# IST-DASLab/gptq-gguf-toolkit

Measured on AMD Instinct MI355X. Metric: Mparams/s GPTQ-quantized, higher is better.
Workload: dtype f32; 1 GPU; llama3-8b-block-q4k: 7 Linears of one block (218.1 M params), 128x2048-token calibration fed per sequence through the package's BlockSchedule, block_size 128, rel_damp 0.01, nstep 20; calib_seqs_per_rank=128, parallelism=calib-dp1+matrix-fanout, owners=rank0

## Files before the change

### gptq-gguf-toolkit_amd/csrc/gq_gemm3p.hpp

```cpp
#pragma once
#include <algorithm>
#include <atomic>
#include <vector>

#include "gq_common.hpp"

namespace gq {
namespace p3 {

constexpr int BLK = 8192;
constexpr int TILE = 256;
constexpr int SLOT_BYTES = 4 * BLK;
constexpr int LDS_BYTES = 4 * SLOT_BYTES;
constexpr int CPT = 8;
typedef float f32x4 __attribute__((ext_vector_type(4)));
typedef unsigned u32x4 __attribute__((ext_vector_type(4)));

__host__ __device__ __forceinline__ unsigned swz(int r) { return (0x78u >> (2 * ((r >> 2) & 3))) & 3u; }

__device__ __forceinline__ void split3(const float (&x)[8], uint4& p1, uint4& p2, uint4& p3) {
    unsigned a[8], b[8], c[8];
#pragma unroll
    for (int e = 0; e < 8; ++e) {
        const unsigned xb = __builtin_bit_cast(unsigned, x[e]);
        const unsigned x1 = xb & 0xffff0000u;
        const float xr = x[e] - __builtin_bit_cast(float, x1);
        const unsigned x2 = __builtin_bit_cast(unsigned, xr) & 0xffff0000u;
        const float xs = xr - __builtin_bit_cast(float, x2);
        a[e] = x1; b[e] = x2; c[e] = __builtin_bit_cast(unsigned, xs);
    }
    p1 = make_uint4(__builtin_amdgcn_perm(a[1], a[0], 0x07060302u), __builtin_amdgcn_perm(a[3], a[2], 0x07060302u),
                    __builtin_amdgcn_perm(a[5], a[4], 0x07060302u), __builtin_amdgcn_perm(a[7], a[6], 0x07060302u));
    p2 = make_uint4(__builtin_amdgcn_perm(b[1], b[0], 0x07060302u), __builtin_amdgcn_perm(b[3], b[2], 0x07060302u),
                    __builtin_amdgcn_perm(b[5], b[4], 0x07060302u), __builtin_amdgcn_perm(b[7], b[6], 0x07060302u));
    p3 = make_uint4(__builtin_amdgcn_perm(c[1], c[0], 0x07060302u), __builtin_amdgcn_perm(c[3], c[2], 0x07060302u),
                    __builtin_amdgcn_perm(c[5], c[4], 0x07060302u), __builtin_amdgcn_perm(c[7], c[6], 0x07060302u));
}
__device__ __forceinline__ float scale_from_max(unsigned maxbits, float& inv) {
    const int ex = (int)((maxbits >> 23) & 0xff);
    int e = (ex == 0 || ex == 0xff) ? 0 : 14 - (ex - 127);
    e = e > 100 ? 100 : (e < -100 ? -100 : e);
    inv = __builtin_bit_cast(float, (unsigned)(127 - e) << 23);
    return __builtin_bit_cast(float, (unsigned)(127 + e) << 23);
}
__device__ __forceinline__ void split2h(const float (&x)[8], float mult, uint4& p1, uint4& p2) {
    unsigned a[4], b[4];
#pragma unroll
    for (int e = 0; e < 4; ++e) {
        unsigned lo[2], hi[2];
#pragma unroll
        for (int u = 0; u < 2; ++u) {
            float v = x[2 * e + u] * mult;
            asm volatile("" : "+v"(v));
            const _Float16 h1 = (_Float16)v;
            float r = v - (float)h1;
            asm volatile("" : "+v"(r));
            const _Float16 h2 = (_Float16)r;
            lo[u] = (unsigned)__builtin_bit_cast(uint16_t, h1);
            hi[u] = (unsigned)__builtin_bit_cast(uint16_t, h2);
        }
        a[e] = lo[0] | (lo[1] << 16);
        b[e] = hi[0] | (hi[1] << 16);
    }
    p1 = make_uint4(a[0], a[1], a[2], a[3]);
    p2 = make_uint4(b[0], b[1], b[2], b[3]);
}

template <int NP, bool TRANS>
__global__ __launch_bounds__(256) void split_kernel(const float* __restrict__ S, int64_t ld, int KC, int tri, int rev,
                                                    unsigned char* __restrict__ img, const unsigned* __restrict__ rmax,
                                                    float* __restrict__ inv_scale) {
    __shared__ float T[TRANS ? 32 : 1][TRANS ? 132 : 1];
    const int c = blockIdx.x, pn = blockIdx.y, tid = threadIdx.x;
    const int kblk = c >> 2;
    const bool zero = (tri == 1 && kblk > pn) || (tri == 2 && kblk < pn);
    if constexpr (TRANS) {
        if (!zero) {
#pragma unroll
            for (int u = 0; u < 4; ++u) {
                const int idx = tid + u * 256, kk = idx >> 5, r4 = (idx & 31) * 4;
                const float4 v = *reinterpret_cast<const float4*>(S + (int64_t)(32 * c + kk) * ld + 128 * pn + r4);
                T[kk][r4] = v.x; T[kk][r4 + 1] = v.y; T[kk][r4 + 2] = v.z; T[kk][r4 + 3] = v.w;
            }
        }
        __syncthreads();
    }
    unsigned char* out = img + ((size_t)pn * KC + (rev ? KC - 1 - c : c)) * (size_t)(NP * BLK);
#pragma unroll
    for (int u = 0; u < 2; ++u) {
        const int p = tid + u * 256, r = p >> 2, kc = (p & 3) ^ (int)swz(r);
        float x[8];
        if (zero) {
#pragma unroll
            for (int e = 0; e < 8; ++e) x[e] = 0.0f;
        } else if constexpr (TRANS) {
#pragma unroll
            for (int e = 0; e < 8; ++e) x[e] = T[8 * kc + e][r];
        } else {
            const float* src = S + (int64_t)(128 * pn + r) * ld + 32 * c + 8 * kc;
            const float4 v0 = *reinterpret_cast<const float4*>(src), v1 = *reinterpret_cast<const float4*>(src + 4);
            x[0] = v0.x; x[1] = v0.y; x[2] = v0.z; x[3] = v0.w; x[4] = v1.x; x[5] = v1.y; x[6] = v1.z; x[7] = v1.w;
        }
        if constexpr (NP == 3) {
            uint4 p1, p2, p3;
            split3(x, p1, p2, p3);
            *reinterpret_cast<uint4*>(out + p * 16) = p1;
            *reinterpret_cast<uint4*>(out + BLK + p * 16) = p2;
            *reinterpret_cast<uint4*>(out + 2 * BLK + p * 16) = p3;
        } else {
            float inv;
            const float mult = scale_from_max(rmax[128 * pn + r], inv);
            if (c == 0 && (p & 3) == 0) inv_scale[128 * pn + r] = inv;
            uint4 p1, p2;
            split2h(x, mult, p1, p2);
            *reinterpret_cast<uint4*>(out + p * 16) = p1;
            *reinterpret_cast<uint4*>(out + BLK + p * 16) = p2;
        }
    }
}

template <bool TRANS>
__global__ __launch_bounds__(256) void row_absmax_kernel(const float* __restrict__ S, int64_t ld, int tri,
                                                         unsigned* __restrict__ rmax) {
    const int kb = blockIdx.x, pn = blockIdx.y, tid = threadIdx.x;
    if ((tri == 1 && kb > pn) || (tri == 2 && kb < pn)) return;
    __shared__ unsigned part[128];
    if (tid < 128) part[tid] = 0u;
    __syncthreads();
    if constexpr (TRANS) {
        float m0 = 0.f, m1 = 0.f, m2 = 0.f, m3 = 0.f;
        const int r4 = (tid & 31) * 4;
#pragma unroll 4
        for (int kk = tid >> 5; kk < 128; kk += 8) {
            const float4 v = *reinterpret_cast<const float4*>(S + (int64_t)(128 * kb + kk) * ld + 128 * pn + r4);
            m0 = fmaxf(m0, fabsf(v.x)); m1 = fmaxf(m1, fabsf(v.y)); m2 = fmaxf(m2, fabsf(v.z)); m3 = fmaxf(m3, fabsf(v.w));
        }
        atomicMax(&part[r4], __builtin_bit_cast(unsigned, m0));
        atomicMax(&part[r4 + 1], __builtin_bit_cast(unsigned, m1));
        atomicMax(&part[r4 + 2], __builtin_bit_cast(unsigned, m2));
        atomicMax(&part[r4 + 3], __builtin_bit_cast(unsigned, m3));
    } else {
        const int r = tid >> 1, h = tid & 1;
        const float* src = S + (int64_t)(128 * pn + r) * ld + 128 * kb + 64 * h;
        float m = 0.f;
#pragma unroll 4
        for (int q = 0; q < 16; ++q) {
            const float4 v = *reinterpret_cast<const float4*>(src + 4 * q);
            m = fmaxf(m, fmaxf(fmaxf(fabsf(v.x), fabsf(v.y)), fmaxf(fabsf(v.z), fabsf(v.w))));
        }
        atomicMax(&part[r], __builtin_bit_cast(unsigned, m));
    }
    __syncthreads();
    if (tid < 128 && part[tid]) atomicMax(&rmax[128 * pn + tid], part[tid]);
}

struct Problem {
    const unsigned char* Aimg;
    const unsigned char* Bimg;
    uint32_t a_panel_bytes, b_panel_bytes;
    float* C;
    int64_t ldc;
    int mode;
    const float* row_scale;
    const float* col_scale;
    float* partial;
};
struct Group {
    Problem p[2];
    const uint32_t* table;
};
constexpr int T_UNITS = 260, NWG = 256;

template <int NP>
__global__ __launch_bounds__(512, 2) void gemm_kernel(const Group g) {
    extern __shared__ __attribute__((aligned(16))) unsigned char smem[];
    const int tid = threadIdx.x, lane = tid & 63;
    const int wid = __builtin_amdgcn_readfirstlane(tid >> 6);
    const int wm = wid >> 2, wn = wid & 3;
    const unsigned qb = g.table[blockIdx.x], qe = g.table[blockIdx.x + 1];
    const unsigned lds0 = (unsigned)(uintptr_t)smem;
    const unsigned ldsw = lds0 + (unsigned)wid * 1024u;
    const int lr = lane & 15, lk = lane >> 4;
    unsigned bA0, bA1, bB0, bB1;
    {
        const unsigned ch = ((unsigned)lk ^ swz(lr)) << 4;
        bA0 = lds0 + (unsigned)(wm * 128 + lr) * 64u + ch;
        bB0 = lds0 + 16384u + (unsigned)(wn * 64 + lr) * 64u + ch;
        bA1 = bA0 + 65536u;
        bB1 = bB0 + 65536u;
    }
    for (unsigned ui = qb; ui < qe; ++ui) {
        __syncthreads();
        const uint32_t* uw = g.table + T_UNITS + 4 * (size_t)ui;
        const uint32_t w0 = (uint32_t)__builtin_amdgcn_readfirstlane((int)uw[0]);
        const int cb = __builtin_amdgcn_readfirstlane((int)uw[1]), ce = __builtin_amdgcn_readfirstlane((int)uw[2]);
        const uint32_t w3 = (uint32_t)__builtin_amdgcn_readfirstlane((int)uw[3]);
        const Problem& P = g.p[w0 >> 28];
        const int tm = (int)((w0 >> 14) & 0x3fff), tn = (int)(w0 & 0x3fff);
        const char* a0 = reinterpret_cast<const char*>(P.Aimg) + (size_t)(2 * tm) * P.a_panel_bytes;
        const char* a1 = a0 + P.a_panel_bytes;
        const char* b0 = reinterpret_cast<const char*>(P.Bimg) + (size_t)(2 * tn) * P.b_panel_bytes;
        const char* b1 = b0 + P.b_panel_bytes;
        const char *a0p0 = a0, *a0p1 = a0 + BLK, *a1p0 = a1, *a1p1 = a1 + BLK;
        const char *b0p0 = b0, *b0p1 = b0 + BLK, *b1p0 = b1, *b1p1 = b1 + BLK;
        const char *a0p2 = a0 + 2 * BLK, *a1p2 = a1 + 2 * BLK, *b0p2 = b0 + 2 * BLK, *b1p2 = b1 + 2 * BLK;
        (void)a0p2; (void)a1p2; (void)b0p2; (void)b1p2;
        constexpr unsigned CH = NP * BLK;
        const unsigned vlast = (unsigned)(ce - 1) * CH + (unsigned)tid * 16u;
        unsigned V0 = (unsigned)cb * CH + (unsigned)tid * 16u, V1, V2, V3, V4;
#define P3_VNEXT()                                               \
    V1 = V0 + CH < vlast ? V0 + CH : vlast;                      \
    V2 = V0 + 2 * CH < vlast ? V0 + 2 * CH : vlast;              \
    V3 = V0 + 3 * CH < vlast ? V0 + 3 * CH : vlast;              \
    V4 = V0 + 4 * CH < vlast ? V0 + 4 * CH : vlast
        P3_VNEXT();
        (void)V3; (void)V4;
#define P3_DL(vo, sp, slot, part)                                                     \
    asm volatile("s_mov_b32 m0, %2\n\ts_nop 0\n\tglobal_load_lds_dwordx4 %0, %1"      \
                 :: "v"(vo), "s"(sp), "s"(ldsw + (unsigned)((slot) * SLOT_BYTES + (part) * BLK)) : "memory")
#define P3_DL4(vo, PA, PB, slot)                                                      \
    P3_DL(vo, a0p##PA, slot, 0); P3_DL(vo, a1p##PA, slot, 1); P3_DL(vo, b0p##PB, slot, 2); P3_DL(vo, b1p##PB, slot, 3)
        f32x4 c00, c01, c02, c03, c10, c11, c12, c13, c20, c21, c22, c23, c30, c31, c32, c33, c40, c41, c42, c43, c50,
            c51, c52, c53, c60, c61, c62, c63, c70, c71, c72, c73;
#define P3_Z(c) c = f32x4{0.f, 0.f, 0.f, 0.f}
        P3_Z(c00); P3_Z(c01); P3_Z(c02); P3_Z(c03); P3_Z(c10); P3_Z(c11); P3_Z(c12); P3_Z(c13);
        P3_Z(c20); P3_Z(c21); P3_Z(c22); P3_Z(c23); P3_Z(c30); P3_Z(c31); P3_Z(c32); P3_Z(c33);
        P3_Z(c40); P3_Z(c41); P3_Z(c42); P3_Z(c43); P3_Z(c50); P3_Z(c51); P3_Z(c52); P3_Z(c53);
        P3_Z(c60); P3_Z(c61); P3_Z(c62); P3_Z(c63); P3_Z(c70); P3_Z(c71); P3_Z(c72); P3_Z(c73);
#undef P3_Z
        u32x4 pa0, pa1, pa2, pa3, pa4, pa5, pa6, pa7, pb0, pb1, pb2, pb3;
        u32x4 qa0, qa1, qa2, qa3, qa4, qa5, qa6, qa7, qb0, qb1, qb2, qb3;
#define P3_DSR(dst, base, off) asm volatile("ds_read_b128 %0, %1 offset:%2" : "=v"(dst) : "v"(base), "n"(off) : "memory")
#define P3_LGKM1(N, x) asm volatile("s_waitcnt lgkmcnt(" #N ")" : "+v"(x)::"memory")
#define P3_LGKM2(N, x, y) asm volatile("s_waitcnt lgkmcnt(" #N ")" : "+v"(x), "+v"(y)::"memory")
#define P3_MF(c, a, b)                                                                                          \
    do {                                                                                                        \
        if constexpr (NP == 3) asm volatile("v_mfma_f32_16x16x32_bf16 %0, %1, %2, %0" : "+v"(c) : "v"(a), "v"(b)); \
        else asm volatile("v_mfma_f32_16x16x32_f16 %0, %1, %2, %0" : "+v"(c) : "v"(a), "v"(b));                 \
    } while (0)
#define P3_STEP(X, Y, AY, BY, OFF, MID, L0, L1, L2, L3)                                               \
    do {                                                                                              \
        P3_LGKM2(10, X##a0, X##b0);                                                                   \
        P3_MF(c00, X##a0, X##b0);                                                                     \
        MID;                                                                                          \
        P3_LGKM1(9, X##b1);                                                                           \
        P3_MF(c01, X##a0, X##b1);                                                                     \
        P3_DSR(Y##a0, AY, (OFF) + 0);                                                                 \
        P3_LGKM1(9, X##b2);                                                                           \
        P3_MF(c02, X##a0, X##b2);                                                                     \
        P3_LGKM1(8, X##b3);                                                                           \
        P3_MF(c03, X##a0, X##b3);                                                                     \
        P3_DSR(Y##b0, BY, (OFF) + 0);                                                                 \
        P3_LGKM1(8, X##a1);                                                                           \
        P3_MF(c10, X##a1, X##b0);                                                                     \
        P3_MF(c11, X##a1, X##b1);                                                                     \
        P3_DSR(Y##b1, BY, (OFF) + 1024);                                                              \
        P3_MF(c12, X##a1, X##b2);                                                                     \
        P3_MF(c13, X##a1, X##b3);                                                                     \
        P3_DSR(Y##b2, BY, (OFF) + 2048);                                                              \
        P3_LGKM1(9, X##a2);                                                                           \
        P3_MF(c20, X##a2, X##b0);                                                                     \
        P3_MF(c21, X##a2, X##b1);                                                                     \
        P3_DSR(Y##b3, BY, (OFF) + 3072);                                                              \
        P3_MF(c22, X##a2, X##b2);                                                                     \
        P3_MF(c23, X##a2, X##b3);                                                                     \
        P3_DSR(Y##a1, AY, (OFF) + 1024);                                                              \
        P3_LGKM1(10, X##a3);                                                                          \
        P3_MF(c30, X##a3, X##b0);                                                                     \
        P3_MF(c31, X##a3, X##b1);                                                                     \
        P3_DSR(Y##a2, AY, (OFF) + 2048);                                                              \
        L0;                                                                                           \
        P3_MF(c32, X##a3, X##b2);                                                                     \
        P3_MF(c33, X##a3, X##b3);                                                                     \
        P3_DSR(Y##a3, AY, (OFF) + 3072);                                                              \
        P3_LGKM1(11, X##a4);                                                                          \
        P3_MF(c40, X##a4, X##b0);                                                                     \
        P3_MF(c41, X##a4, X##b1);                                                                     \
        P3_DSR(Y##a4, AY, (OFF) + 4096);                                                              \
        L1;                                                                                           \
        P3_MF(c42, X##a4, X##b2);                                                                     \
        P3_MF(c43, X##a4, X##b3);                                                                     \
        P3_DSR(Y##a5, AY, (OFF) + 5120);                                                              \
        P3_LGKM1(12, X##a5);                                                                          \
        P3_MF(c50, X##a5, X##b0);                                                                     \
        P3_MF(c51, X##a5, X##b1);                                                                     \
        P3_DSR(Y##a6, AY, (OFF) + 6144);                                                              \
        L2;                                                                                           \
        P3_MF(c52, X##a5, X##b2);                                                                     \
        P3_MF(c53, X##a5, X##b3);                                                                     \
        P3_DSR(Y##a7, AY, (OFF) + 7168);                                                              \
        P3_LGKM1(13, X##a6);                                                                          \
        P3_MF(c60, X##a6, X##b0);                                                                     \
        P3_MF(c61, X##a6, X##b1);                                                                     \
        L3;                                                                                           \
        P3_MF(c62, X##a6, X##b2);                                                                     \
        P3_MF(c63, X##a6, X##b3);                                                                     \
        P3_LGKM1(12, X##a7);                                                                          \
        P3_MF(c70, X##a7, X##b0);                                                                     \
        P3_MF(c71, X##a7, X##b1);                                                                     \
        P3_MF(c72, X##a7, X##b2);                                                                     \
        P3_MF(c73, X##a7, X##b3);                                                                     \
    } while (0)
#define P3_IV0(VO, PA, PB)                                                                                        \
    P3_STEP(p, q, bA0, bB0, 32768, asm volatile("s_waitcnt vmcnt(4)\n\ts_barrier" ::: "memory"), P3_DL(VO, a0p##PA, 3, 0), \
            P3_DL(VO, a1p##PA, 3, 1), P3_DL(VO, b0p##PB, 3, 2), P3_DL(VO, b1p##PB, 3, 3))
#define P3_IV1(VO, PA, PB)                                                                                        \
// ... 166 lines not shown
    const int slot_base = 0;
    struct Tile { int prob, tm, tn, len; };
    std::vector<Tile> tiles;
    struct Blk { int neg_len, prob, bi, bj; };
    std::vector<Blk> blocks;
    for (int prob = 0; prob < (int)shapes.size(); ++prob) {
        const GemmShape& s = shapes[prob];
        const bool by_m = s.kr == 3;
        const int bm = by_m ? 4 : 8, bn = by_m ? 8 : 4;
        const int nbm = (s.MT + bm - 1) / bm, nbn = (s.NT + bn - 1) / bn;
        for (int bi = 0; bi < nbm; ++bi)
            for (int bj = 0; bj < nbn; ++bj) {
                int mx = 0;
                for (int tm = bi * bm; tm < std::min(s.MT, (bi + 1) * bm); ++tm)
                    for (int tn = bj * bn; tn < std::min(s.NT, (bj + 1) * bn); ++tn)
                        if (!s.lower || tm >= tn) mx = std::max(mx, tile_len(s, tm, tn));
                if (mx > 0) blocks.push_back({-mx, prob, bi, bj});
            }
    }
    std::stable_sort(blocks.begin(), blocks.end(), [](const Blk& a, const Blk& b) { return a.neg_len < b.neg_len; });
    for (auto& b : blocks) {
        const GemmShape& s = shapes[b.prob];
        const bool by_m = s.kr == 3;
        const int bm = by_m ? 4 : 8, bn = by_m ? 8 : 4;
        for (int tm = b.bi * bm; tm < std::min(s.MT, (b.bi + 1) * bm); ++tm)
            for (int tn = b.bj * bn; tn < std::min(s.NT, (b.bj + 1) * bn); ++tn)
                if (!s.lower || tm >= tn) {
                    const int len = tile_len(s, tm, tn);
                    if (len > 0) tiles.push_back({b.prob, tm, tn, len});
                }
    }
    struct Piece { int tile, cb, ce; };
    long total = 0;
    for (auto& t : tiles) total += t.len + OVH;
    std::vector<Piece> seg[8];
    {
        long acc = 0;
        int x = 0;
        for (int ti = 0; ti < (int)tiles.size(); ++ti) {
            int at = 0;
            const int len = tiles[ti].len;
            while (at < len) {
                const long end_x = (x == 7) ? (long)1 << 60 : (total * (x + 1)) / 8;
                long room = end_x - acc - OVH;
                int take = len - at;
                if (room < take) {
                    int r = (int)std::max<long>(room, 0) / gran * gran;
                    if (r < MINP) r = 0;
                    if (take - r < MINP) r = take;
                    take = r;
                }
                if (take > 0) {
                    seg[x].push_back({ti, at, at + take});
                    acc += take + OVH;
                    at += take;
                }
                if (at < len || acc >= end_x) {
                    if (x < 7) ++x;
                    else if (take == 0) { seg[x].push_back({ti, at, len}); acc += len - at + OVH; at = len; }
                }
            }
        }
    }
    std::vector<Piece> wg[NWG];
    double mk = 0;
    for (int x = 0; x < 8; ++x) {
        long tot = 0;
        for (auto& p : seg[x]) tot += p.ce - p.cb + OVH;
        std::vector<Piece> mine[32];
        long load[32];
        for (long T = (tot + 31) / 32;; T += gran) {
            for (int w = 0; w < 32; ++w) { load[w] = 0; mine[w].clear(); }
            size_t done = 0;
            while (done + 32 <= seg[x].size()) {
                bool ok = true;
                for (int w = 0; w < 32 && ok; ++w) {
                    const Piece& p = seg[x][done + w];
                    ok = load[w] + (p.ce - p.cb) + OVH <= T;
                }
                if (!ok) break;
                for (int w = 0; w < 32; ++w) {
                    const Piece& p = seg[x][done + w];
                    load[w] += p.ce - p.cb + OVH;
                    mine[w].push_back(p);
                }
                done += 32;
            }
            int w = 0;
            bool fits = true;
            for (size_t i = done; i < seg[x].size() && fits; ++i) {
                Piece p = seg[x][i];
                while (p.cb < p.ce) {
                    if (w > 31) { fits = false; break; }
                    const int len = p.ce - p.cb;
                    const long room = T - load[w] - OVH;
                    int take;
                    if (room >= len) take = len;
                    else {
                        take = (int)(std::max<long>(room, 0) / gran * gran);
                        if (len - take < MINP) take = (len - MINP) / gran * gran;
                        if (take < MINP) { ++w; continue; }
                    }
                    mine[w].push_back({p.tile, p.cb, p.cb + take});
                    load[w] += take + OVH;
                    p.cb += take;
                }
            }
            if (fits) break;
        }
        for (int w = 0; w < 32; ++w) {
            wg[w * 8 + x] = mine[w];
            mk = std::max(mk, (double)load[w]);
        }
    }
    std::vector<int> npieces(tiles.size(), 0), first_slot(tiles.size(), -1), seen(tiles.size(), 0);
    for (int b = 0; b < NWG; ++b)
        for (auto& p : wg[b]) ++npieces[p.tile];
    Plan pl;
    int slots = 0;
    for (size_t t = 0; t < tiles.size(); ++t)
        if (npieces[t] > 1) {
            first_slot[t] = slot_base + slots;
            slots += npieces[t];
            pl.rlist.push_back((uint32_t)tiles[t].prob << 28 | (uint32_t)tiles[t].tm << 14 | (uint32_t)tiles[t].tn);
            pl.rlist.push_back((uint32_t)first_slot[t] << 8 | (uint32_t)npieces[t]);
        }
    pl.nslots = slots;
    pl.table.assign(T_UNITS, 0u);
    unsigned at = 0;
    for (int b = 0; b < NWG; ++b) {
        pl.table[b] = at;
        for (auto& p : wg[b]) {
            const Tile& t = tiles[p.tile];
            pl.table.push_back((uint32_t)t.prob << 28 | (uint32_t)t.tm << 14 | (uint32_t)t.tn);
            pl.table.push_back((uint32_t)p.cb);
            pl.table.push_back((uint32_t)p.ce);
            pl.table.push_back(npieces[p.tile] > 1 ? (uint32_t)(first_slot[p.tile] + seen[p.tile]++ + 1) : 0u);
            ++at;
        }
    }
    pl.table[NWG] = at;
    pl.makespan = mk;
    pl.ideal = (double)total / NWG;
    if (slots > max_slots) pl.nslots = -1;
    return pl;
}

template <int NP>
inline int launch_split(bool trans, const float* S, int64_t ld, int64_t R, int64_t K, int tri, int rev, unsigned char* img,
                        unsigned* rmax, float* inv_scale, hipStream_t st) {
    const dim3 grid((unsigned)(K / 32), (unsigned)(R / 128)), block(256);
    ProfScope ps(PT_CHOL_SPLIT, st);
    if constexpr (NP == 2) {
        GQ_HIP(hipMemsetAsync(rmax, 0, (size_t)R * 4, st));
        const dim3 g2((unsigned)(K / 128), (unsigned)(R / 128));
        if (trans) hipLaunchKernelGGL(row_absmax_kernel<true>, g2, block, 0, st, S, ld, tri, rmax);
        else hipLaunchKernelGGL(row_absmax_kernel<false>, g2, block, 0, st, S, ld, tri, rmax);
        GQ_LAUNCH_CHECK();
    }
    if (trans) hipLaunchKernelGGL((split_kernel<NP, true>), grid, block, 0, st, S, ld, (int)(K / 32), tri, rev, img, rmax, inv_scale);
    else hipLaunchKernelGGL((split_kernel<NP, false>), grid, block, 0, st, S, ld, (int)(K / 32), tri, rev, img, rmax, inv_scale);
    GQ_LAUNCH_CHECK();
    return GQ_OK;
}

template <int NP>
inline int launch_gemm(const Group& g, int n_reduce, const uint32_t* rlist_dev, hipStream_t st) {
    static std::atomic<bool> attr_set{false};
    if (!attr_set) {
        GQ_HIP(hipFuncSetAttribute((const void*)gemm_kernel<NP>, hipFuncAttributeMaxDynamicSharedMemorySize, LDS_BYTES));
        attr_set = true;
    }
    ProfScope ps(PT_CHOL_IMG_GEMM, st);
    hipLaunchKernelGGL(gemm_kernel<NP>, dim3(256), dim3(512), LDS_BYTES, st, g);
    GQ_LAUNCH_CHECK();
    if (n_reduce > 0) {
        hipLaunchKernelGGL(reduce_kernel<NP>, dim3((unsigned)n_reduce, 16), dim3(256), 0, st, g, rlist_dev);
        GQ_LAUNCH_CHECK();
    }
    return GQ_OK;
}

}
}
```

### gptq-gguf-toolkit_amd/csrc/gq_gptq.hip

```cpp
#include <atomic>
#include <mutex>
#include "gq_common.hpp"
#include "gq_gemm32.hpp"
#include "gq_walk.hpp"
#include <stdlib.h>

namespace gq {

constexpr int SEG = 128;
constexpr int SB = 16;
constexpr int SEG_WAVES = 8;
constexpr int SEG_LDS_BYTES = (SEG * 64 + SEG * SEG + 2 * SB * 64) * 4 + SEG * 8;

__device__ __forceinline__ float div_rcp64(float n, double rd) { return (float)((double)n * rd); }

struct BandTable {
    int32_t n;
    int32_t end64[GQ_BANDS_MAX];
    uint32_t info[GQ_BANDS_MAX];
    int64_t sm_off[GQ_BANDS_MAX];
};
template <bool BANDS> struct BandArg {};
template <> struct BandArg<true> { BandTable t; };

// ... 476 lines not shown
    case WalkKind::Bands:
        hipLaunchKernelGGL((gptq_segment_kernel<false, false, true>), grid, block, SEG_LDS_BYTES, c.st, c.W, c.C, src, ld_src,
                           c.U, a, len, c.R, c.d, c.s, c.dmin, c.m, 0, 0, 0.0f, 0.0f, c.qweight, b.Err, ldE, err_col0, nullptr,
                           nullptr, nullptr, unext, npair, BandArg<true>{c.bands->tbl});
        break;
    case WalkKind::Uniform:
        hipLaunchKernelGGL((gptq_segment_kernel<false, true>), grid, block, SEG_LDS_BYTES, c.st, c.W, c.C, src, ld_src, c.U, a,
                           len, c.R, c.d, c.s, c.dmin, c.m, ti.group, 0, 0.0f, (float)ti.qmax, c.qweight, b.Err, ldE, err_col0,
                           nullptr, c.uni.scale, c.uni.zero, unext);
        break;
    case WalkKind::ActOrder:
        hipLaunchKernelGGL(gptq_segment_kernel<true>, grid, block, SEG_LDS_BYTES, c.st, c.W, c.C, src, ld_src, c.U, a, len, c.R,
                           c.d, c.s, c.dmin, c.m, ti.group, ti.is_signed, (float)ti.qmin, (float)ti.qmax, c.qweight, b.Err, ldE,
                           err_col0, c.perm, nullptr, nullptr, unext, npair);
        break;
    case WalkKind::KQuant:
        hipLaunchKernelGGL(gptq_segment_kernel<false>, grid, block, SEG_LDS_BYTES, c.st, c.W, c.C, src, ld_src, c.U, a, len, c.R,
                           c.d, c.s, c.dmin, c.m, ti.group, ti.is_signed, (float)ti.qmin, (float)ti.qmax, c.qweight, b.Err, ldE,
                           err_col0, nullptr, nullptr, nullptr, unext, npair);
        break;
    }
    GQ_LAUNCH_CHECK();
    return GQ_OK;
}

static int walk_block(const Walk& w, const Block& b, bool& walked_by_partner) {
    const WalkCall& c = w.c;
    const int64_t B = w.p.B;
    int rc;
    if (!b.single) {
        ProfScope ps(PT_BLOCK_FAR, c.st);
        hipLaunchKernelGGL(copy2d_kernel, dim3(2048), dim3(256), 0, c.st, w.Wblk, B, c.W + b.c1, c.C, c.R, b.c2 - b.c1);
        GQ_LAUNCH_CHECK();
    }
    int64_t a = walked_by_partner ? b.c2 : b.c1;
    walked_by_partner = false;
    while (a < b.c2) {
        int64_t e = a + SEG < b.c2 ? a + SEG : b.c2;
        const int64_t next_sg = (a / 256 + 1) * 256;
        if (e > next_sg) e = next_sg;
        const int len = (int)(e - a);
        if (w.search == ScaleSearch::Lazy && (a % 256) == 0 && (rc = lazy_search(w, a))) return rc;
        const float* unext =
            (w.p.pair_look && b.single && len == SEG && !(b.pos & 1) && b.c2 + B <= c.C) ? c.U + a * c.C + a + SEG : nullptr;
        const int npair = (unext && c.kind != WalkKind::Uniform && B == SEG) ? 2 : 1;
        walked_by_partner = npair == 2;
        if ((rc = launch_segment(w, b, a, len, unext, npair))) return rc;
        if (e < b.c2) {
            ProfScope ps(PT_BLOCK_FAR, c.st);
            hipLaunchKernelGGL(block_far_update_kernel, dim3(2048), dim3(256), 0, c.st, w.Wblk + (e - b.c1), B, b.c2 - e, c.R,
                               b.Err, w.p.ldE, a - b.c1, len, c.U, c.C, a, e);
            GQ_LAUNCH_CHECK();
        }
        a = e;
    }
    return GQ_OK;
}


static int block_trailing_update(const Walk& w, const Block& b, int64_t end) {
    const WalkCall& c = w.c;
    return launch_trailing_update(c.W + b.c2, c.C, b.Err + b.pos * w.p.B, w.p.ldE, c.U + b.c1 * c.C + b.c2, c.C, c.R,
                                  end - b.c2, b.c2 - b.c1, c.st);
}

static int pair_near_update(const Walk& w, const Block& b) {
    if (!(b.pos & 1)) return GQ_OK;
    const WalkCall& c = w.c;
    const int64_t B = w.p.B, n = b.S1 - b.c2;
    const float *E = b.Err + (b.pos - 1) * B, *Up = c.U + (b.c1 - B) * c.C + b.c2;
    ProfScope ps(PT_TRAILING, c.st);
    if (n <= w.p.near64_maxn && c.R % 64 == 0) return launch_gemm32_near256(c.W + b.c2, c.C, E, w.p.ldE, Up, c.C, c.R, n, c.st);
    return launch_gemm32<false, 0, false, 0, LA_B>(c.W + b.c2, c.C, E, w.p.ldE, Up, c.C, c.R, n, 2 * B, c.st);
}

static int far_update(const Walk& w, const Block& b) {
    const WalkCall& c = w.c;
    ProfScope ps(PT_TRAILING_FAR, c.st);
    return launch_gemm32<false, 0, false, 0, LA_B>(c.W + b.S1, c.C, b.Err, w.p.ldE, c.U + b.S0 * c.C + b.S1, c.C, c.R,
                                                   c.C - b.S1, b.S1 - b.S0, c.st);
}

struct FarHelper {
    hipStream_t st = nullptr;
    hipEvent_t done = nullptr;
    bool enqueueing = false, recorded = false;
};
static std::mutex g_far_mu;
static FarHelper g_far[64];
static int far_helper_acquire(FarHelper** out) {
    *out = nullptr;
    int dev = 0;
    GQ_HIP(hipGetDevice(&dev));
    std::lock_guard<std::mutex> lk(g_far_mu);
    FarHelper& h = g_far[dev & 63];
    if (!h.st) {
        GQ_HIP(hipStreamCreateWithFlags(&h.st, hipStreamNonBlocking));
        GQ_HIP(hipEventCreateWithFlags(&h.done, hipEventDisableTiming));
    }
    if (h.enqueueing) return GQ_OK;
    if (h.recorded && hipEventQuery(h.done) != hipSuccess) {
        (void)hipGetLastError();
        return GQ_OK;
    }
    h.enqueueing = true;
    *out = &h;
    return GQ_OK;
}
static void far_helper_release(FarHelper* h) {
    if (!h) return;
    std::lock_guard<std::mutex> lk(g_far_mu);
    h->recorded = hipEventRecord(h->done, h->st) == hipSuccess;
    h->enqueueing = false;
}
struct FarHold {
    FarHelper* h = nullptr;
    ~FarHold() { far_helper_release(h); }
};
static int far_event(int i, hipEvent_t* out) {
    thread_local hipEvent_t pool[96] = {};
    hipEvent_t& e = pool[i % 96];
    if (!e) GQ_HIP(hipEventCreateWithFlags(&e, hipEventDisableTiming));
    *out = e;
    return GQ_OK;
}

struct FarPipeline {
    FarHold hold;
    hipStream_t helper = nullptr;
    hipEvent_t ev_small_prev = nullptr;
    hipEvent_t ev_bulk[2] = {nullptr, nullptr};
    hipEvent_t ev_last = nullptr;
    int ev_i = 0;

    int lease() {
        int rc;
        if ((rc = far_helper_acquire(&hold.h))) return rc;
        if (hold.h) helper = hold.h->st;
        return GQ_OK;
    }
    int wait_for_half(hipStream_t st, int64_t sb) {
        if (!ev_bulk[sb & 1]) return GQ_OK;
        GQ_HIP(hipStreamWaitEvent(st, ev_bulk[sb & 1], 0));
        ev_bulk[sb & 1] = nullptr;
        return GQ_OK;
    }
    int far_update(const Walk& w, const Block& b) {
        const WalkCall& c = w.c;
        const int64_t C = c.C, S0 = b.S0, S1 = b.S1, ldE = w.p.ldE, K = S1 - S0;
        const int64_t G = (int64_t)w.p.la * w.p.B, g1 = S1 + G < C ? S1 + G : C, g2 = g1 + G < C ? g1 + G : C;
        const float* Us = c.U + S0 * C;
        hipEvent_t ready = nullptr, ev = nullptr;
        int rc;
        if (g1 < C) {
            if ((rc = far_event(ev_i++, &ready))) return rc;
            GQ_HIP(hipEventRecord(ready, c.st));
        }
        if (ev_small_prev) GQ_HIP(hipStreamWaitEvent(c.st, ev_small_prev, 0));
        ev_small_prev = nullptr;
        {
            ProfScope ps(PT_TRAILING_FAR, c.st);
            if ((rc = launch_gemm32_chain_full<LA_B>(c.W + S1, C, b.Err, ldE, Us + S1, C, c.R, g1 - S1, K, c.st))) return rc;
        }
        if (g1 >= C) return GQ_OK;
        GQ_HIP(hipStreamWaitEvent(helper, ready, 0));
        ProfScope ps(PT_TRAILING_FAR, helper);
        if ((rc = launch_gemm32_chain_full<LA_B>(c.W + g1, C, b.Err, ldE, Us + g1, C, c.R, g2 - g1, K, helper, w.p.far_wgs)))
            return rc;
        if ((rc = far_event(ev_i++, &ev))) return rc;
        GQ_HIP(hipEventRecord(ev, helper));
        ev_small_prev = ev;
        if (g2 < C &&
            (rc = launch_gemm32_chain_full<LA_B>(c.W + g2, C, b.Err, ldE, Us + g2, C, c.R, C - g2, K, helper, w.p.far_wgs)))
            return rc;
        if ((rc = far_event(ev_i++, &ev))) return rc;
        GQ_HIP(hipEventRecord(ev, helper));
        ev_bulk[b.sb & 1] = ev;
        ev_last = ev;
        return GQ_OK;
    }
    int final_wait(hipStream_t st) {
        if (ev_last) GQ_HIP(hipStreamWaitEvent(st, ev_last, 0));
        return GQ_OK;
    }
};

static int column_walk(const WalkCall& c) {
    Walk w{c};
    int rc;
    if ((rc = walk_open(c, w))) return rc;
    const WalkPlan& p = w.p;
    FarPipeline far;
    if (p.helper_ok) {
        if ((rc = far.lease())) return rc;
        w.helper = far.helper != nullptr;
    }
    if ((w.ti.k_search && w.search != ScaleSearch::None) || c.researches_out) GQ_HIP(hipMemsetAsync(w.panel, 0, 256, c.st));
    if (c.kind == WalkKind::Uniform && c.uni.group <= 0) {
        uniform_params(w, 0, (int)c.C, 0);
        GQ_LAUNCH_CHECK();
    }
    if (w.search == ScaleSearch::UpFront && (rc = up_front_search(w))) return rc;
    if ((rc = segment_attributes())) return rc;

    bool walked_by_partner = false;
    for (int64_t c1 = 0; c1 < c.C; c1 += p.B) {
        Block b;
        b.c1 = c1;
        b.c2 = c1 + p.B < c.C ? c1 + p.B : c.C;
        b.single = (b.c2 - b.c1) <= SEG && (b.c1 / 256 == (b.c2 - 1) / 256);
        const int64_t bi = c1 / p.B;
        b.sb = bi / p.la;
        b.pos = p.lookahead ? bi % p.la : 0;
        b.S0 = b.sb * p.la * p.B;
        b.S1 = b.S0 + p.la * p.B < c.C ? b.S0 + p.la * p.B : c.C;
        b.Err = w.err[w.helper ? b.sb & 1 : 0];
        if (w.helper && b.pos == 0 && (rc = far.wait_for_half(c.st, b.sb))) return rc;
        if (c.kind == WalkKind::Uniform && c.uni.group > 0 && (rc = uniform_grids(w, b))) return rc;
        if ((rc = walk_block(w, b, walked_by_partner))) return rc;
        if (b.c2 >= c.C) break;
        if (!p.lookahead) rc = block_trailing_update(w, b, c.C);
        else if (b.c2 < b.S1) rc = p.pair_look ? pair_near_update(w, b) : block_trailing_update(w, b, b.S1);
        else rc = w.helper ? far.far_update(w, b) : far_update(w, b);
        if (rc) return rc;
    }
    if ((rc = far.final_wait(c.st))) return rc;
    if (c.researches_out)
        GQ_HIP(hipMemcpyAsync(c.researches_out, w.panel + GQ_PANEL_RESEARCH, sizeof(int32_t), hipMemcpyDeviceToDevice, c.st));
    return GQ_OK;
}

static WalkCall walk_call(WalkKind kind, float* W, const float* U, int64_t R, int64_t C, int block_size, uint8_t* qweight,
                          void* ws, size_t ws_bytes, hipStream_t st) {
    WalkCall c;
    c.kind = kind;
    c.W = W, c.U = U, c.R = R, c.C = C, c.block_size = block_size;
    c.qweight = qweight;
    c.ws = ws, c.ws_bytes = ws_bytes, c.st = st;
    return c;
}

int gptq_quantize(float* W, const float* U, int64_t R, int64_t C, int q_type, int block_size, int static_groups,
                  const gq_search_t* p, uint8_t* qweight, uint16_t* d, uint8_t* s, uint16_t* dmin, uint8_t* m,
                  void* ws, size_t ws_bytes, hipStream_t st, const int32_t* perm, const int64_t* row_ends, int nstack,
                  int32_t* researches_out) {
    if (nstack > 1 && perm) GQ_FAIL(GQ_E_UNSUPPORTED, "gq_gptq_quantize_stacked: act_order matrices are not stacked");
    WalkCall c = walk_call(perm ? WalkKind::ActOrder : WalkKind::KQuant, W, U, R, C, block_size, qweight, ws, ws_bytes, st);
    c.d = d, c.s = s, c.dmin = dmin, c.m = m;
    c.q_type = q_type;
    c.static_groups = static_groups != 0;
    c.p = p;
    c.row_ends = row_ends, c.nstack = nstack, c.researches_out = researches_out;
    c.perm = perm;
    return column_walk(c);
}

int gptq_quantize_bands(float* W, const float* U, int64_t R, int64_t C, const gq_band_t* bands_host, int n_bands,
                        int block_size, const gq_search_t* p, uint8_t* qweight, uint16_t* d, uint8_t* s, uint16_t* dmin,
                        uint8_t* m, void* ws, size_t ws_bytes, hipStream_t st) {
    if (!bands_host) GQ_FAIL(GQ_E_NULL, "gq_gptq_quantize_bands: null band table");
    if (n_bands < 1 || n_bands > GQ_BANDS_MAX)
        GQ_FAIL(GQ_E_BAD_SHAPE, "gq_gptq_quantize_bands: %d bands (1..%d)", n_bands, GQ_BANDS_MAX);
    if (R <= 0 || C <= 0 || C % 256) GQ_FAIL(GQ_E_BAD_SHAPE, "gq_gptq_quantize_bands: R=%ld C=%ld (C %% 256 != 0)", (long)R, (long)C);
    BandPlan bp{};
    bp.tbl.n = n_bands;
    int64_t prev = 0, off = 0;
    for (int k = 0; k < n_bands; ++k) {
        const int64_t e = bands_host[k].row_end;
        TypeInfo tk;
        if (!type_info(bands_host[k].q_type, tk))
            GQ_FAIL(GQ_E_BAD_TYPE, "gq_gptq_quantize_bands: band %d has unknown q_type %d", k, (int)bands_host[k].q_type);
        if (e % 64 || e <= prev || e > R || e / 64 > INT32_MAX)
            GQ_FAIL(GQ_E_BAD_SHAPE, "gq_gptq_quantize_bands: band %d ends at row %ld (ascending multiples of 64 up to R=%ld)", k,
                    (long)e, (long)R);
        bp.q_type[k] = bands_host[k].q_type;
        bp.row_end[k] = e;
        bp.tbl.end64[k] = (int32_t)(e / 64);
        bp.tbl.info[k] = (uint32_t)tk.group | (uint32_t)tk.is_signed << 8 | (uint32_t)(uint8_t)(int8_t)tk.qmin << 16 |
                         (uint32_t)tk.qmax << 24;
        bp.tbl.sm_off[k] = off;
        off += (e - prev) * (C / tk.group);
        prev = e;
    }
    if (prev != R) GQ_FAIL(GQ_E_BAD_SHAPE, "gq_gptq_quantize_bands: the last band ends at row %ld, R=%ld", (long)prev, (long)R);
    WalkCall c = walk_call(WalkKind::Bands, W, U, R, C, block_size, qweight, ws, ws_bytes, st);
    c.d = d, c.s = s, c.dmin = dmin, c.m = m;
    c.p = p;
    c.bands = &bp;
    return column_walk(c);
}

int obq_quantize(float* W, const float* U, int64_t R, int64_t C, int bits, int group_size, int sym, int block_size,
                 uint8_t* qweight, float* scale, float* zero, void* ws, size_t ws_bytes, hipStream_t st) {
    if (bits < 1 || bits > 8) GQ_FAIL(GQ_E_UNSUPPORTED, "gq_obq_quantize: bits=%d (1..8: qweight is uint8)", bits);
    if (!scale || !zero) GQ_FAIL(GQ_E_NULL, "gq_obq_quantize: null pointer");
    if (group_size < 0 || (group_size > 0 && (group_size % SB || C % group_size)))
        GQ_FAIL(GQ_E_UNSUPPORTED, "gq_obq_quantize: group_size %d must be 0 or a multiple of 16 that divides C=%ld", group_size, (long)C);
    WalkCall c = walk_call(WalkKind::Uniform, W, U, R, C, block_size, qweight, ws, ws_bytes, st);
    c.uni = UniformSpec{bits, group_size, sym ? 1 : 0, scale, zero};
    return column_walk(c);
}

}
```

Measured before the change: 2458 Mparams/s.

## Fuse row absmax and split into one row-staged kernel for non-transposed 2-plane images

For the two-plane, non-transposed case with K up to 8192, a new kernel stages four full rows in LDS. It computes each row's absmax with a wave reduction and then writes the split image, replacing the memset, the row_absmax kernel and the split kernel. This removes two launches, the atomics, and a second read of S from global memory, at the cost of a large LDS footprint (about 128 KB at K=8192), which limits occupancy. Separately, the far-update 'ready' event is now recorded after the near trailing GEMM instead of before it, so the helper stream waits for that GEMM. Two profiling scripts are also added.

```diff
diff --git a/gptq-gguf-toolkit_amd/csrc/gq_gemm3p.hpp b/gptq-gguf-toolkit_amd/csrc/gq_gemm3p.hpp
--- a/gptq-gguf-toolkit_amd/csrc/gq_gemm3p.hpp
+++ b/gptq-gguf-toolkit_amd/csrc/gq_gemm3p.hpp
@@ -152,6 +152,65 @@
     }
     __syncthreads();
     if (tid < 128 && part[tid]) atomicMax(&rmax[128 * pn + tid], part[tid]);
+}
+
+constexpr int IMAGE_ROWS_MAX_K = 8192;
+__host__ __device__ __forceinline__ int image_rows_stride(int K) { return (K + 255) & ~255; }
+inline size_t image_rows_lds(int K) { return (size_t)image_rows_stride(K) * 16 + 16; }
+__global__ __launch_bounds__(256) void image_rows_kernel(const float* __restrict__ S, int64_t ld, int K, int tri, int rev,
+                                                         unsigned char* __restrict__ img, float* __restrict__ inv_scale) {
+    extern __shared__ __attribute__((aligned(16))) unsigned char rows_smem[];
+    const int Kp = image_rows_stride(K);
+    float* rows = reinterpret_cast<float*>(rows_smem);
+    unsigned* smax = reinterpret_cast<unsigned*>(rows + 4 * Kp);
+    const int tid = threadIdx.x, lane = tid & 63, w = tid >> 6;
+    const int r0 = 4 * (int)blockIdx.x, pn = r0 >> 7, rp = r0 & 127;
+    const int KC = K >> 5;
+    const int j_lo = tri == 2 ? 32 * pn : 0, j_hi = tri == 1 ? (32 * (pn + 1) < K / 4 ? 32 * (pn + 1) : K / 4) : K / 4;
+    const int t_end = Kp >> 8, t_lo = j_lo < j_hi ? j_lo >> 6 : t_end, t_hi = j_lo < j_hi ? (j_hi + 63) >> 6 : t_end;
+    {
+        const float* src = S + (int64_t)(r0 + w) * ld;
+        float4* dst = reinterpret_cast<float4*>(rows + (size_t)w * Kp);
+        const float4 zero4 = make_float4(0.f, 0.f, 0.f, 0.f);
+        for (int t = 0; t < t_lo; ++t) dst[lane + 64 * t] = zero4;
+        for (int t = t_hi; t < t_end; ++t) dst[lane + 64 * t] = zero4;
+        float m = 0.f;
+        for (int tb = t_lo; tb < t_hi; tb += 8) {
+            float4 v[8];
+#pragma unroll
+            for (int u = 0; u < 8; ++u) {
+                const int j = lane + 64 * (tb + u), jc = j < j_lo ? j_lo : (j >= j_hi ? j_hi - 1 : j);
+                v[u] = *reinterpret_cast<const float4*>(src + 4 * jc);
+                if (j != jc) v[u] = zero4;
+            }
+#pragma unroll
+            for (int u = 0; u < 8; ++u) {
+                m = fmaxf(m, fmaxf(fmaxf(fabsf(v[u].x), fabsf(v[u].y)), fmaxf(fabsf(v[u].z), fabsf(v[u].w))));
+                if (tb + u < t_hi) dst[lane + 64 * (tb + u)] = v[u];
+            }
+        }
+#pragma unroll
+        for (int o = 32; o >= 1; o >>= 1) m = fmaxf(m, __shfl_xor(m, o));
+        if (lane == 0) smax[w] = __builtin_bit_cast(unsigned, m);
+    }
+    __syncthreads();
+    const int q = lane & 3, hi = lane >> 2, row = hi >> 2, half = (hi >> 1) & 1;
+    const int r = rp + row, kc = q ^ (int)swz(r);
+    float inv;
+    const float mult = scale_from_max(smax[row], inv);
+    if (w == 0 && (hi & 3) == 0 && q == 0) inv_scale[r0 + row] = inv;
+    const float* lrow = rows + (size_t)row * Kp + 8 * kc;
+    for (int c = 4 * w + (hi & 3); c < KC; c += 16) {
+        const float4 va = *reinterpret_cast<const float4*>(lrow + 32 * c + 4 * half);
+        const float4 vb = *reinterpret_cast<const float4*>(lrow + 32 * c + 4 * (half ^ 1));
+        const float4 v0 = half ? vb : va, v1 = half ? va : vb;
+        const float x[8] = {v0.x, v0.y, v0.z, v0.w, v1.x, v1.y, v1.z, v1.w};
+        uint4 p1, p2;
+        split2h(x, mult, p1, p2);
+        unsigned char* out = img + ((size_t)pn * KC + (rev ? KC - 1 - c : c)) * (size_t)(2 * BLK) + (r * 4 + q) * 16;
+        *reinterpret_cast<uint4*>(out) = p1;
+        *reinterpret_cast<uint4*>(out + BLK) = p2;
+    }
 }
 
 struct Problem {
@@ -624,6 +683,18 @@
     const dim3 grid((unsigned)(K / 32), (unsigned)(R / 128)), block(256);
     ProfScope ps(PT_CHOL_SPLIT, st);
     if constexpr (NP == 2) {
+        if (!trans && K <= IMAGE_ROWS_MAX_K) {
+            static std::atomic<bool> attr_set{false};
+            if (!attr_set) {
+                GQ_HIP(hipFuncSetAttribute((const void*)image_rows_kernel, hipFuncAttributeMaxDynamicSharedMemorySize,
+                                           (int)image_rows_lds(IMAGE_ROWS_MAX_K)));
+                attr_set = true;
+            }
+            hipLaunchKernelGGL(image_rows_kernel, dim3((unsigned)(R / 4)), block, image_rows_lds((int)K), st, S, ld, (int)K, tri, rev,
+                               img, inv_scale);
+            GQ_LAUNCH_CHECK();
+            return GQ_OK;
+        }
         GQ_HIP(hipMemsetAsync(rmax, 0, (size_t)R * 4, st));
         const dim3 g2((unsigned)(K / 128), (unsigned)(R / 128));
         if (trans) hipLaunchKernelGGL(row_absmax_kernel<true>, g2, block, 0, st, S, ld, tri, rmax);
diff --git a/gptq-gguf-toolkit_amd/csrc/gq_gptq.hip b/gptq-gguf-toolkit_amd/csrc/gq_gptq.hip
--- a/gptq-gguf-toolkit_amd/csrc/gq_gptq.hip
+++ b/gptq-gguf-toolkit_amd/csrc/gq_gptq.hip
@@ -652,10 +652,6 @@
         const float* Us = c.U + S0 * C;
         hipEvent_t ready = nullptr, ev = nullptr;
         int rc;
-        if (g1 < C) {
-            if ((rc = far_event(ev_i++, &ready))) return rc;
-            GQ_HIP(hipEventRecord(ready, c.st));
-        }
         if (ev_small_prev) GQ_HIP(hipStreamWaitEvent(c.st, ev_small_prev, 0));
         ev_small_prev = nullptr;
         {
@@ -663,6 +659,8 @@
             if ((rc = launch_gemm32_chain_full<LA_B>(c.W + S1, C, b.Err, ldE, Us + S1, C, c.R, g1 - S1, K, c.st))) return rc;
         }
         if (g1 >= C) return GQ_OK;
+        if ((rc = far_event(ev_i++, &ready))) return rc;
+        GQ_HIP(hipEventRecord(ready, c.st));
         GQ_HIP(hipStreamWaitEvent(helper, ready, 0));
         ProfScope ps(PT_TRAILING_FAR, helper);
         if ((rc = launch_gemm32_chain_full<LA_B>(c.W + g1, C, b.Err, ldE, Us + g1, C, c.R, g2 - g1, K, helper, w.p.far_wgs)))
diff --git a/profiles/widest_chain_probe.py b/profiles/widest_chain_probe.py
--- /dev/null
+++ b/profiles/widest_chain_probe.py
@@ -0,0 +1,30 @@
+#!/usr/bin/env python3
+import json, os, statistics, sys, time
+import torch
+sys.path.insert(0, os.path.dirname(os.path.dirname(os.path.abspath(__file__))))
+from gptq_gguf_toolkit_amd import ops, _cabi
+Q4_K = 12
+R, C, N = 4096, 14336, int(os.environ.get("N", 10))
+torch.manual_seed(0)
+T = 2 * C
+X = (torch.randn(T, C, device="cuda") * torch.exp(torch.randn(C, device="cuda") * 0.5)).half()
+H0 = torch.zeros(C, C, device="cuda")
+ops.h_accumulate(H0, X, 0.0, 2.0 / 8)
+del X
+W0 = torch.randn(R, C, device="cuda") * 0.02
+_cabi.prof_enable([])
+prep, loop = [], []
+for it in range(N + 2):
+    H = H0.clone(); W = W0.clone(); torch.cuda.synchronize()
+    t0 = time.perf_counter()
+    U, flag = ops.h_prepare(H, W, 0.01)
+    torch.cuda.synchronize(); t1 = time.perf_counter()
+    out = ops.gptq_quantize(W, U, Q4_K, 128)
+    torch.cuda.synchronize(); t2 = time.perf_counter()
+    if it >= 2:
+        prep.append(1e3 * (t1 - t0)); loop.append(1e3 * (t2 - t1))
+import zlib
+crc = zlib.crc32(U.cpu().numpy().tobytes()) ^ zlib.crc32(out[0].cpu().numpy().tobytes())
+print(json.dumps({"tag": os.environ.get("TAG"), "prep_min": round(min(prep), 3), "prep_med": round(statistics.median(prep), 3),
+                  "loop_min": round(min(loop), 3), "loop_med": round(statistics.median(loop), 3), "flag": int(flag.item()),
+                  "helper": bool(ops.uses_helper_stream(R, C, 128)), "crc": crc}))
diff --git a/profiles/widest_chain_trace.py b/profiles/widest_chain_trace.py
--- /dev/null
+++ b/profiles/widest_chain_trace.py
@@ -0,0 +1,27 @@
+#!/usr/bin/env python3
+import csv, glob, sys
+d = sys.argv[1]
+f = glob.glob(d + "/**/*kernel_trace.csv", recursive=True)[0]
+rows = list(csv.DictReader(open(f)))
+name = [k for k in rows[0] if k.lower() == "kernel_name"][0]
+st = [k for k in rows[0] if k.lower().startswith("start")][0]
+en = [k for k in rows[0] if k.lower().startswith("end")][0]
+rows.sort(key=lambda r: int(r[st]))
+idx = max(i for i, r in enumerate(rows) if "equil_kernel" in r[name])
+last = rows[idx:]
+span = (max(int(r[en]) for r in last) - int(last[0][st])) / 1e6
+print(f"last iteration: {len(last)} kernels, span {span:.2f} ms (from equil_kernel)")
+agg = {}
+for r in last:
+    n = r[name]
+    a = agg.setdefault(n, [0, 0.0]); a[0] += 1; a[1] += (int(r[en]) - int(r[st])) / 1e3
+for n, (c, us) in sorted(agg.items(), key=lambda kv: -kv[1][1]):
+    print(f"{n[:90]:90s} {c:5d} {us/1e3:9.3f} ms {us/c:9.1f} us")
+far = [(int(r[en]) - int(r[st])) / 1e3 for r in last if "gemm32_chain_full_kernel" in r[name]]
+print("far-next launches in order (us):", " ".join(f"{x:.0f}" for x in far))
+segs = [r for r in last if "gptq_segment_kernel" in r[name]]
+if segs:
+    t_first = int(segs[0][st]); t_last = max(int(r[en]) for r in last)
+    print(f"column loop (first segment kernel -> last kernel): {(t_last - t_first)/1e6:.2f} ms")
+    hp = (t_first - int(last[0][st])) / 1e6
+    print(f"h_prepare (equil_kernel -> first segment kernel): {hp:.2f} ms")
```

Result: faster. 2487 Mparams/s, median of 6 (+1.2%).
